# SeekStorm/SeekStorm

Measured on NVIDIA B200. Metric: queries/sec at top-10 (1M x 768 f32 cosine brute-force kNN), higher is better.
Workload: dtype f32

## Files before the change

### include/seekstorm_b200.h

```cpp
#ifndef SEEKSTORM_B200_H
#define SEEKSTORM_B200_H
#include <stdint.h>
#include <stddef.h>

#ifdef __cplusplus
extern "C" {
#endif

#define SSB_ABI_VERSION 3
#define SSB_K_MAX 32u
#define SSB_K_LIMIT 1024u
#define SSB_MAX_QUERY_TERMS 32u

enum { SSB_OK = 0, SSB_E_INVALID = -1, SSB_E_CUDA = -2, SSB_E_NOMEM = -3, SSB_E_STATE = -4,
       SSB_E_UNSUPPORTED = -5, SSB_E_NO_DEVICE = -6 };

enum { SSB_QUERY_UNION = 0, SSB_QUERY_INTERSECTION = 1, SSB_QUERY_PHRASE = 2 };
enum { SSB_RESULT_COUNT = 0, SSB_RESULT_TOPK = 1, SSB_RESULT_TOPKCOUNT = 2 };
enum { SSB_SIM_DOT = 0, SSB_SIM_COSINE = 1, SSB_SIM_EUCLIDEAN = 2 };
enum { SSB_QUANT_NONE = 0, SSB_QUANT_SCALAR_I8 = 1,
       SSB_QUANT_TURBO_I8 = 2 };
enum { SSB_VEC_KERNEL_AUTO = 0, SSB_VEC_KERNEL_FFMA = 1, SSB_VEC_KERNEL_TCGEN05 = 2, SSB_VEC_KERNEL_TCGEN05_N64 = 3,
       SSB_VEC_KERNEL_TCGEN05_BF16 = 4, SSB_VEC_KERNEL_TCGEN05_BF16_N64 = 5,
       SSB_VEC_KERNEL_TCGEN05_BF16_N256 = 6 ,
// ... 132 lines not shown
#define SSB_COMM_ID_BYTES 128
int32_t ssb_comm_unique_id(uint8_t* id128);
int32_t ssb_comm_init(ssb_index* ix, const uint8_t* id128, uint32_t rank, uint32_t world);
int32_t ssb_comm_attach(ssb_index* ix, void* nccl_comm, uint32_t rank, uint32_t world);
int32_t ssb_comm_destroy(ssb_index* ix);
int32_t ssb_lexical_sync_df(ssb_index* ix);

int32_t ssb_sync(ssb_index* ix);
void*   ssb_stream(ssb_index* ix);
#define SSB_OWN_STREAM ((void*)(intptr_t)-1)
int32_t ssb_set_stream(ssb_index* ix, void* cuda_stream);

typedef struct {
    uint64_t kernel_launches;
    uint64_t algorithmic_bytes;
    uint64_t h2d_bytes, d2h_bytes;
    uint64_t postings_visited;
    uint64_t probes;
    uint64_t items_processed;
    uint64_t items_skipped;
    uint64_t dominant_kernel_ns;
    uint64_t scan_bytes_read;
    uint64_t filter_fallbacks;
    uint64_t reserved[1];
} ssb_stats;
int32_t ssb_last_stats(const ssb_index* ix, ssb_stats* out);

#ifdef __cplusplus
}
#endif
#endif
```

### seekstorm_b200/_lib.py

```python
from __future__ import annotations

import ctypes as C
import os

_HERE = os.path.dirname(os.path.abspath(__file__))
LIB_PATH = os.environ.get("SSB_LIB") or os.path.join(_HERE, "libseekstorm_b200.so")

SSB_OK = 0
K_MAX = 32
MAX_QUERY_TERMS = 32

QUERY_UNION, QUERY_INTERSECTION, QUERY_PHRASE = 0, 1, 2
RESULT_COUNT, RESULT_TOPK, RESULT_TOPKCOUNT = 0, 1, 2
SIM_DOT, SIM_COSINE, SIM_EUCLIDEAN = 0, 1, 2


class SsbHit(C.Structure):
    _fields_ = [("doc_id", C.c_uint64), ("score", C.c_float), ("pad", C.c_uint32)]


class SsbConfig(C.Structure):
    _fields_ = [("device", C.c_int32), ("max_batch", C.c_uint32), ("vector_dims", C.c_uint32),
                ("vector_similarity", C.c_uint32), ("vector_kernel", C.c_uint32), ("vector_quantization", C.c_uint32),
                ("reserved", C.c_uint32 * 2)]


class SsbHitExt(C.Structure):
    _fields_ = [("field_id", C.c_uint32), ("chunk_id", C.c_uint32), ("level_id", C.c_uint32), ("shard_id", C.c_uint32),
                ("cluster_id", C.c_uint32), ("cluster_score", C.c_float), ("vector_score", C.c_float),
                ("lexical_score", C.c_float), ("source", C.c_uint32), ("pad", C.c_uint32 * 3)]


class SsbVecQuery(C.Structure):
# ... 18 lines not shown
                ("term_keys", C.c_void_p), ("term_flags", C.c_void_p),
                ("filter_offsets", C.c_void_p), ("filters", C.c_void_p), ("filter_set_values", C.c_void_p),
                ("field_masks", C.c_void_p)]


class SsbFacetField(C.Structure):
    _fields_ = [("type", C.c_uint32), ("offset", C.c_uint32)]


class SsbFacetFilter(C.Structure):
    _fields_ = [("facet", C.c_uint32), ("kind", C.c_uint32), ("start", C.c_uint64), ("end", C.c_uint64),
                ("set_first", C.c_uint32), ("set_count", C.c_uint32)]


FACET_U8, FACET_U16, FACET_U32, FACET_U64, FACET_I8, FACET_I16, FACET_I32, FACET_I64, FACET_TIMESTAMP, FACET_F32, FACET_F64, \
    FACET_STRING16, FACET_STRING32 = range(13)
FILTER_RANGE, FILTER_SET = 0, 1


class SsbStats(C.Structure):
    _fields_ = [("kernel_launches", C.c_uint64), ("algorithmic_bytes", C.c_uint64), ("h2d_bytes", C.c_uint64),
                ("d2h_bytes", C.c_uint64), ("postings_visited", C.c_uint64), ("probes", C.c_uint64),
                ("items_processed", C.c_uint64), ("items_skipped", C.c_uint64), ("dominant_kernel_ns", C.c_uint64),
                ("scan_bytes_read", C.c_uint64), ("filter_fallbacks", C.c_uint64), ("reserved", C.c_uint64 * 1)]


EXPORTS = [
    "ssb_abi_version", "ssb_last_error", "ssb_create", "ssb_destroy", "ssb_lexical_add_level",
    "ssb_vector_add_level_clustered", "ssb_lexical_set_field_boosts", "ssb_lexical_commit", "ssb_lexical_dict_size", "ssb_lexical_dict_export", "ssb_lexical_set_global_df",
    "ssb_load_index_bin", "ssb_load_vector_bin", "ssb_index_bin_inspect", "ssb_set_deleted", "ssb_set_facets", "ssb_vector_set_turboquant_mask", "ssb_vector_add_level", "ssb_vector_count", "ssb_vector_reserve", "ssb_set_vector_kernel", "ssb_search_lexical", "ssb_search_vector", "ssb_search_vector_ex", "ssb_search_hybrid",
    "ssb_rrf_fuse", "ssb_comm_unique_id", "ssb_comm_init", "ssb_comm_attach", "ssb_comm_destroy", "ssb_lexical_sync_df",
    "ssb_search_vector_keys", "ssb_search_lexical_keys", "ssb_merge_keys", "ssb_sync",
    "ssb_stream", "ssb_set_stream", "ssb_last_stats",
]

_lib = None


class SsbError(RuntimeError):
    pass


def lib():
    global _lib
    if _lib is not None:
        return _lib
    if not os.path.exists(LIB_PATH):
# ... 57 lines not shown
```

### seekstorm_b200/csrc/api.cu

```cuda
#include <stdarg.h>
#include <string.h>
#include <algorithm>
#include <condition_variable>
#include <exception>
#include <memory>
#include <mutex>
#include <new>
#include <shared_mutex>
#include <vector>

#include "bm25.h"
#include "comm.h"
#include "common.cuh"
#include "vec_scan.h"

namespace ssb {

static thread_local char g_err[512] = "";

void set_error(const char* fmt, ...) {
    va_list ap; va_start(ap, fmt);
    vsnprintf(g_err, sizeof(g_err), fmt, ap);
    va_end(ap);
}
// ... 200 lines not shown
        SSB_TRY(c.qlo.reserve((size_t)nq_pad * ix->dpad, 0, st));
        if (filter) SSB_TRY(c.q_scale.reserve(nq_pad, 0, st));
        SSB_TRY(vec::launch_prep_split_queries_bf16((const float*)qsrc, nq, ix->dims, ix->dims, c.qhi.p, c.qlo.p, nq_pad, ix->dpad,
                                                    ix->cfg.vector_similarity == SSB_SIM_COSINE, st, (filter || ivf) ? c.qpad.p : nullptr,
                                                    filter ? c.q_scale.p : nullptr, filter ? ix->vec_err.p : nullptr));
    } else
    SSB_TRY(vec::launch_prep_queries((const float*)qsrc, nq, ix->dims, ix->dims, c.qpad.p, nq_pad, ix->dpad,
                                     ix->cfg.vector_similarity == SSB_SIM_COSINE, st));
    c.stats.kernel_launches += 1;
    if (ix->n_rows == 0) { SSB_CUDA_TRY(cudaMemsetAsync(keys_out_dev, 0, (size_t)nq * LIST * 8, st)); return SSB_OK; }
    size_t sb = use_tc ? vec::scan_tc_scratch_bytes(ix->n_sms, nq_pad) : vec::scan_scratch_bytes(ix->n_sms, nq_pad);
    const size_t head_words = sb / 8 + (size_t)nq_pad * LIST + (nq_pad + 1) / 2;
    SSB_TRY(c.scratch.reserve(head_words + (filter ? vec::refine_scratch_words(ix->n_sms, nq_pad) : 0), 0, st));
    vec::ScanArgs a{};
    a.rows = ix->rows.p; a.rows_hi = ix->rows_hi.p; a.rows_lo = ix->rows_lo.p; a.rows_h16 = ix->rows_h16.p; a.doc_ids = ix->doc_ids.p; a.n_rows = ix->n_rows; a.dpad = ix->dpad; a.queries_padded = c.qpad.p;
    a.nq_pad = nq_pad; a.nq_valid = nq; a.k = k; a.similarity = ix->cfg.vector_similarity; a.n_sms = ix->n_sms;
    a.scratch = c.scratch.p; a.scratch_bytes = sb;
    uint64_t* merged = c.scratch.p + sb / 8;
    a.keys_out = merged; a.ev0 = c.ev0; a.ev1 = c.ev1; c.ev_used = true;
    a.thr_buf = reinterpret_cast<uint32_t*>(merged + (size_t)nq_pad * LIST);
    a.ceil_keys = ceil_dev;
    if (ix->del.n) { a.del_slot = ix->del.d_slot; a.del_words = ix->del.d_words; }
    a.launches = &c.stats.kernel_launches;
    if (ivf) {
        vec::IvfArgs v{};
        v.medoids = ix->medoids.p; v.lvl_begin = ix->lvl_begin.p; v.cl_count = ix->cl_count.p;
        v.n_clusters = ix->n_clusters; v.n_levels = (uint32_t)ix->h_lvl_begin.size(); v.max_level_clusters = ix->max_level_clusters;
        v.queries_padded = c.qpad.p; v.nq = nq; v.nq_pad = nq_pad; v.dpad = ix->dpad; v.similarity = ix->cfg.vector_similarity;
        v.ann_mode = ivf->mode; v.n_probe = ivf->n_probe; v.cluster_threshold = ivf->thr;
        v.words = (ix->n_clusters + 31) / 32;
        SSB_TRY(c.ivf_scores.reserve((size_t)nq * ix->n_clusters, 0, st));
        SSB_TRY(c.ivf_sel.reserve((size_t)nq_pad * v.words, 0, st));
        SSB_TRY(c.ivf_obs.reserve(nq, 0, st));
        v.scores = c.ivf_scores.p; v.sel = c.ivf_sel.p; v.observed = c.ivf_obs.p; v.launches = &c.stats.kernel_launches;
        SSB_TRY(vec::launch_ivf_select(v, st));
        a.ivf_sel = c.ivf_sel.p; a.ivf_words = v.words; a.row_cluster = ix->row_cluster.p;
    }
    if (ix->quant_i8) {
        a.rows_i8 = ix->rows_i8.p; a.queries_i8 = c.q_i8.p; a.dpad8 = ix->dpad8;
        if (ix->turbo || ix->cfg.vector_similarity != SSB_SIM_COSINE) {
            a.i8_scaled = ix->cfg.vector_similarity == SSB_SIM_EUCLIDEAN ? (ix->affine ? 3 : 2) : 1;
            a.row_aff = ix->row_aff.p; a.q_aff = c.q_aff.p;
            a.row_scale = ix->row_scale.p; a.row_norm = ix->row_norm.p; a.q_scale = c.q_scale.p; a.q_norm = c.q_norm.p;
        }
        SSB_TRY(vec::launch_scan_tc(a, 128, 2, st));
    } else if (use_tc) {
        SSB_TRY(c.qhi.reserve((size_t)nq_pad * ix->dpad, 0, st));
        SSB_TRY(c.qlo.reserve((size_t)nq_pad * ix->dpad, 0, st));
        a.q_hi = c.qhi.p; a.q_lo = c.qlo.p;
        if (filter) a.q_scale = c.q_scale.p;
        SSB_TRY(vec::launch_scan_tc(a, qt, filter ? (kern == SSB_VEC_KERNEL_TCGEN05_FILTER_N256_PAIR ? 4 : 3) : (tc_bf16 ? 1 : 0), st));
        if (filter) {
            vec::RefineArgs r{};
            r.rows = ix->rows.p; r.doc_ids = ix->doc_ids.p; r.n_rows = ix->n_rows; r.dpad = ix->dpad; r.queries_padded = c.qpad.p; r.margin = c.q_scale.p;
            r.keys = merged; r.keys_out = keys_out_dev;
            r.nq = nq; r.nq_pad = nq_pad; r.k = k;
            r.fb_lists = c.scratch.p + head_words;
            r.fb_state = reinterpret_cast<uint32_t*>(r.fb_lists + (size_t)nq_pad * ix->n_sms * LIST);
            r.del_slot = a.del_slot; r.del_words = a.del_words; r.ivf_sel = a.ivf_sel; r.ivf_words = a.ivf_words; r.row_cluster = a.row_cluster; r.n_sms = ix->n_sms; r.launches = &c.stats.kernel_launches;
            SSB_TRY(vec::launch_refine(r, st));
            c.fb_state = r.fb_state;
        }
    } else {
        SSB_TRY(vec::launch_scan_ffma(a, st));
    }
    if (!filter) SSB_CUDA_TRY(cudaMemcpyAsync(keys_out_dev, merged, (size_t)nq * LIST * 8, cudaMemcpyDeviceToDevice, st));
    c.stats.algorithmic_bytes += (uint64_t)(nq_pad / qt) * ix->n_rows * ix->dims * (ix->quant_i8 ? 1 : 4);
    c.stats.scan_bytes_read += filter ? (uint64_t)(nq_pad / qt) * ix->n_rows * ix->dims * 2 + (uint64_t)nq * LIST * ix->dims * 4
                                      : (uint64_t)(nq_pad / qt) * ix->n_rows * ix->dims * (ix->quant_i8 ? 1 : 4);
    return SSB_OK;
}

uint32_t decode_list(const uint64_t* keys, uint32_t k, ssb_hit* hits, bool dedup) {
    uint32_t n = 0;
    for (uint32_t j = 0; j < LIST && n < k; j++) {
        const uint64_t key = keys[j];
        if (!key) break;
        const uint64_t doc = key_doc(key);
        if (dedup) { bool seen = false; for (uint32_t i = 0; i < n; i++) seen = seen || hits[i].doc_id == doc; if (seen) continue; }
        hits[n].doc_id = doc; hits[n].score = key_score(key); hits[n].pad = 0;
        n++;
    }
    return n;
}

void decode_keys(const uint64_t* keys, uint32_t nq, uint32_t k, ssb_hit* hits, uint32_t* n_hits, bool dedup = false) {
    for (uint32_t q = 0; q < nq; q++) {
        const uint32_t n = decode_list(keys + (size_t)q * LIST, k, hits + (size_t)q * k, dedup);
        for (uint32_t j = n; j < k; j++) { hits[(size_t)q * k + j].doc_id = 0; hits[(size_t)q * k + j].score = 0.f; hits[(size_t)q * k + j].pad = 0; }
// ... 895 lines not shown
```

### seekstorm_b200/csrc/vec_refine.cu

```cuda
#include "common.cuh"
#include "vec_scan.h"

namespace ssb {
namespace vec {
namespace rf {

constexpr int RTHREADS = 128;
constexpr int QF = 4;
constexpr int FTHREADS = 256;

__device__ __forceinline__ float dot4(const float4 a, const float4 b, float s) {
    s = fmaf(a.x, b.x, s); s = fmaf(a.y, b.y, s); s = fmaf(a.z, b.z, s); return fmaf(a.w, b.w, s);
}

__global__ void __launch_bounds__(RTHREADS)
refine_candidates(const float* __restrict__ rows, const uint32_t* __restrict__ doc_ids, uint32_t dpad, const float* __restrict__ queries,
                  const float* __restrict__ margin, const uint64_t* keys, uint64_t* keys_out, uint32_t k, uint32_t* __restrict__ fb_state) {
    __shared__ uint64_t ex[LIST];
    const int warp = threadIdx.x >> 5, lane = threadIdx.x & 31;
    const uint32_t q = blockIdx.x;
    const uint64_t mine = keys[(size_t)q * LIST + lane];
    const float* qv = queries + (size_t)q * dpad;
    uint64_t ck[8]; const float* rp[8]; float s[8];
#pragma unroll
    for (int c = 0; c < 8; c++) {
        ck[c] = shfl64(mine, warp * 8 + c);
        rp[c] = rows + (size_t)(ck[c] ? key_doc(ck[c]) : 0u) * dpad;
        s[c] = 0.f;
    }
    if (ck[0]) {
        for (uint32_t i = lane * 4; i < dpad; i += 128) {
            const float4 b = *reinterpret_cast<const float4*>(qv + i);
#pragma unroll
            for (int c = 0; c < 8; c++) s[c] = dot4(__ldg(reinterpret_cast<const float4*>(rp[c] + i)), b, s[c]);
        }
    }
#pragma unroll
    for (int c = 0; c < 8; c++) {
        float v = s[c];
        for (int m = 16; m; m >>= 1) v += __shfl_xor_sync(FULL, v, m);
        if (lane == 0) {
            uint64_t key = 0;
            if (ck[c] && v == v) { const uint32_t row = key_doc(ck[c]); key = pack_key(v, doc_ids ? __ldg(&doc_ids[row]) : row); }
            ex[warp * 8 + c] = key;
        }
    }
    __syncthreads();
    if (warp == 0) {
        keys_out[(size_t)q * LIST + lane] = wl_sort_desc(ex[lane], lane);
        const uint64_t kth = shfl64(mine, (int)k - 1), last = shfl64(mine, LIST - 1);
        if (lane == 0 && last && kth) {
            const float m = margin[q], th = __fsub_rd(key_score(kth), m);
            if (!(m == m) || key_score(last) >= th) fb_state[1 + atomicAdd(&fb_state[0], 1u)] = q;
        }
    }
}

__global__ void __launch_bounds__(FTHREADS)
fallback_scan(const float* __restrict__ rows, const uint32_t* __restrict__ doc_ids, uint64_t n_rows, uint32_t dpad,
              const float* __restrict__ queries, const uint32_t* __restrict__ fb_state, uint64_t* __restrict__ fb_lists ,
              uint32_t k, const uint32_t* __restrict__ del_slot, const uint64_t* __restrict__ del_words,
              const uint32_t* __restrict__ ivf_sel, uint32_t ivf_words, const uint32_t* __restrict__ row_cluster) {
    const uint32_t nf = fb_state[0];
    if (nf == 0) return;
    extern __shared__ __align__(16) float qs[];
    __shared__ uint64_t sm[FTHREADS / 32][QF][LIST];
    const int warp = threadIdx.x >> 5, lane = threadIdx.x & 31;
    for (uint32_t base = 0; base < nf; base += QF) {
        for (uint32_t i = threadIdx.x; i < QF * dpad; i += FTHREADS) {
            const uint32_t j = i / dpad;
            qs[i] = base + j < nf ? queries[(size_t)fb_state[1 + base + j] * dpad + (i - j * dpad)] : 0.f;
        }
        __syncthreads();
        uint64_t L[QF];
#pragma unroll
        for (int j = 0; j < QF; j++) L[j] = 0;
        for (uint64_t row = (uint64_t)blockIdx.x * (FTHREADS / 32) + warp; row < n_rows; row += (uint64_t)gridDim.x * (FTHREADS / 32)) {
// ... 31 lines not shown
}

__global__ void __launch_bounds__(32)
fallback_merge(const uint32_t* __restrict__ fb_state, const uint64_t* __restrict__ fb_lists, uint32_t n_lists, uint64_t* __restrict__ keys) {
    const uint32_t nf = fb_state[0];
    const int lane = threadIdx.x;
    for (uint32_t slot = blockIdx.x; slot < nf; slot += gridDim.x) {
        uint64_t L = 0;
        for (uint32_t l = 0; l < n_lists; l++) {
            const uint64_t B = fb_lists[((size_t)slot * n_lists + l) * LIST + lane];
            if (__any_sync(FULL, B != 0)) L = wl_merge(L, B, lane);
        }
        keys[(size_t)fb_state[1 + slot] * LIST + lane] = L;
    }
}

}

size_t refine_scratch_words(int n_sms, uint32_t nq_pad) { return (size_t)nq_pad * (size_t)n_sms * LIST + (nq_pad + 2) / 2 + 1; }

int32_t launch_refine(const RefineArgs& a, cudaStream_t st) {
    if (a.nq == 0) return SSB_OK;
    SSB_CUDA_TRY(cudaMemsetAsync(a.fb_state, 0, 4, st));
    rf::refine_candidates<<<a.nq, rf::RTHREADS, 0, st>>>(a.rows, a.doc_ids, a.dpad, a.queries_padded, a.margin, a.keys, a.keys_out, a.k, a.fb_state);
    SSB_CUDA_TRY(cudaGetLastError());
    const int smem = rf::QF * (int)a.dpad * 4;
    if (smem > 200 * 1024) { set_error("filter scan: vector_dims too large for the fallback scan"); return SSB_E_UNSUPPORTED; }
    if (smem > 40 * 1024) SSB_CUDA_TRY(cudaFuncSetAttribute(rf::fallback_scan, cudaFuncAttributeMaxDynamicSharedMemorySize, smem));
    rf::fallback_scan<<<a.n_sms, rf::FTHREADS, smem, st>>>(a.rows, a.doc_ids, a.n_rows, a.dpad, a.queries_padded, a.fb_state, a.fb_lists, a.k,
                                                           a.del_slot, a.del_words, a.ivf_sel, a.ivf_words, a.row_cluster);
    SSB_CUDA_TRY(cudaGetLastError());
    rf::fallback_merge<<<64, 32, 0, st>>>(a.fb_state, a.fb_lists, (uint32_t)a.n_sms, a.keys_out);
    SSB_CUDA_TRY(cudaGetLastError());
    if (a.launches) *a.launches += 3;
    return SSB_OK;
}

}
}
```

### seekstorm_b200/csrc/vec_scan.h

```cpp
#pragma once
#include <cuda_runtime.h>
#include <stdint.h>

namespace ssb {
namespace vec {

constexpr int VEC_QT = 16;

struct ScanArgs {
    const float* rows;
    const void* rows_hi = nullptr; const void* rows_lo = nullptr;
    const void* rows_h16 = nullptr;
    const uint32_t* doc_ids;
    uint64_t n_rows;
    uint32_t dpad;
    const float* queries_padded;
    uint32_t nq_pad;
    uint32_t nq_valid = 0;
    uint32_t k;
    uint32_t similarity;
    int n_sms;
    uint64_t* scratch;
    size_t scratch_bytes;
    uint64_t* keys_out;
    cudaEvent_t ev0 = nullptr, ev1 = nullptr;
    float* q_hi = nullptr; float* q_lo = nullptr;
    uint32_t* thr_buf = nullptr;
    const uint32_t* thr_init = nullptr;
    const uint64_t* ceil_keys = nullptr;
    uint64_t* launches = nullptr;
    const int8_t* rows_i8 = nullptr;
    const int8_t* queries_i8 = nullptr;
    uint32_t dpad8 = 0;
    int i8_scaled = 0;
    const float* row_scale = nullptr; const float* row_norm = nullptr;
    const float* q_scale = nullptr; const float* q_norm = nullptr;
    const int* row_aff = nullptr; const int* q_aff = nullptr;
    const uint32_t* del_slot = nullptr; const uint64_t* del_words = nullptr;
    bool sample_groupmax = false;
    const uint32_t* ivf_sel = nullptr; uint32_t ivf_words = 0; const uint32_t* row_cluster = nullptr;
};

inline uint64_t vec_presample_rows(uint64_t n_rows, bool tensor_core) {
    if (n_rows < 65536) return 0;
    uint64_t s = tensor_core ? n_rows / 128 : n_rows / 32;
    const uint64_t lo = tensor_core ? 2048 : 4096, hi = tensor_core ? 8192 : 32768;
    s = s < lo ? lo : (s > hi ? hi : s);
    return s / 512 * 512;
}

int32_t launch_scan_ffma(const ScanArgs& a, cudaStream_t st);
size_t scan_scratch_bytes(int n_sms, uint32_t nq_pad);
int32_t launch_scan_tc(const ScanArgs& a, uint32_t nq_tile , int prec , cudaStream_t st);
size_t scan_tc_scratch_bytes(int n_sms, uint32_t nq_pad);
int32_t launch_prep_split_queries_bf16(const float* q, uint32_t nq, uint32_t dims, uint64_t qstride, void* hi, void* lo, uint32_t nq_pad,
                                       uint32_t dpad, int normalize, cudaStream_t st, float* f32_out = nullptr, float* margin_out = nullptr,
                                       const uint32_t* row_err = nullptr);
int32_t launch_rows_f16_err(const float* rows, void* h16, uint64_t n, uint32_t dpad, float scale, uint32_t* err, cudaStream_t st);
int32_t launch_max_abs_f32(const float* x, size_t n, uint32_t* out_bits, cudaStream_t st);
struct RefineArgs {
    const float* rows; const uint32_t* doc_ids; uint64_t n_rows; uint32_t dpad;
    const float* queries_padded;
    const float* margin;
    const uint64_t* keys;
    uint64_t* keys_out;
    uint32_t nq, nq_pad, k;
    uint32_t* fb_state;
    uint64_t* fb_lists;
    const uint32_t* del_slot; const uint64_t* del_words;
    const uint32_t* ivf_sel; uint32_t ivf_words; const uint32_t* row_cluster;
    int n_sms;
    uint64_t* launches;
};
struct IvfArgs {
    const float* medoids;
    const uint32_t* lvl_begin;
    const uint32_t* cl_count;
    uint32_t n_clusters, n_levels, max_level_clusters;
    const float* queries_padded;
    uint32_t nq, nq_pad, dpad, similarity;
    uint32_t ann_mode, n_probe; float cluster_threshold;
    float* scores;
    uint32_t* sel; uint32_t words;
    uint64_t* observed;
    uint64_t* launches;
};
int32_t launch_ivf_select(const IvfArgs& a, cudaStream_t st);
// ... 26 lines not shown
```

### seekstorm_b200/csrc/vec_scan_tc.cu

```cuda
#include <cuda_bf16.h>
#include <stdlib.h>
#include <cuda_fp16.h>

#include "common.cuh"
#include "vec_scan.h"

namespace ssb {
namespace vec {

namespace tc {
constexpr int KC = 32;
constexpr int TM = 128;
constexpr int MT = 2;
constexpr int TROWS = TM * MT;
constexpr int A1_BYTES = TM * KC * 4;
constexpr int A_BYTES = MT * A1_BYTES;
constexpr int THREADS = 512;
constexpr int SPLIT_THREADS = 256;
constexpr int CHUNK = 8;
enum { PREC_TF32 = 0, PREC_BF16 = 1, PREC_I8 = 2, PREC_F16F = 3 };

constexpr int MAX_STAGES = 6;
template <int NQ, int PREC, bool BRES = false> struct Cfg {
    static constexpr int MT = NQ == 256 ? 1 : 2;
// ... 576 lines not shown
                        else while (pm) { const int src = __ffs(pm) - 1; pm &= pm - 1; wl_insert(L, shfl64(key, src), lane); }
                        mylists[q * LIST + lane] = L;
                        uint32_t kth = (uint32_t)(shfl64(L, (int)k - 1) >> 32);
                        if (kth) kth = ord_f32(__fsub_rd(unord_f32(kth), qs_sm[q]));
                        if (lane == 0 && kth > thr_u[q]) atomicMax(&thr_u[q], kth);
                    }
                }
            }
            tc_fence_before();
            __syncwarp();
            if (lane == 0) mbar_arrive_leader(&tempty[buf]);
        }
    }

    tc_fence_before();
    __syncthreads();
    cluster_sync_all();
    if (warp == 1) {
        tc_fence_after();
        asm volatile("tcgen05.dealloc.cta_group::2.sync.aligned.b32 %0, %1;" ::"r"(tmem_base), "r"((uint32_t)C::TMEM_COLS) : "memory");
    }
}

__global__ void split_queries_tf32(const float* __restrict__ q, float* __restrict__ hi, float* __restrict__ lo, size_t n) {
    size_t i = (size_t)blockIdx.x * blockDim.x + threadIdx.x;
    if (i >= n) return;
    uint32_t x = __float_as_uint(q[i]), h = x & 0xFFFFE000u;
    hi[i] = __uint_as_float(h);
    lo[i] = __uint_as_float(x) - __uint_as_float(h);
}
__global__ void prep_split_queries_bf16(const float* __restrict__ q, uint32_t nq, uint32_t dims, uint64_t qstride,
                                        __nv_bfloat16* __restrict__ hi, __nv_bfloat16* __restrict__ lo, uint32_t nq_pad, uint32_t dpad, int normalize,
                                        float* __restrict__ f32_out ,
                                        float* __restrict__ margin_out , const uint32_t* __restrict__ row_err ) {
    const int lane = threadIdx.x & 31;
    const uint32_t row = blockIdx.x * (blockDim.x >> 5) + (threadIdx.x >> 5);
    if (row >= nq_pad) return;
    const bool filter = margin_out != nullptr;
    __nv_bfloat16* oh = hi + (size_t)row * dpad;
    __nv_bfloat16* ol = lo + (size_t)row * dpad;
    __half* o16 = reinterpret_cast<__half*>(oh);
    float* of = f32_out ? f32_out + (size_t)row * dpad : nullptr;
    if (row >= nq) {
        for (uint32_t i = lane; i < dpad; i += 32) { oh[i] = __float2bfloat16_rn(0.f); if (!filter) ol[i] = __float2bfloat16_rn(0.f); if (of) of[i] = 0.f; }
        if (filter && lane == 0) margin_out[row] = 0.f;
        return;
// ... 178 lines not shown
    SSB_TRY(encode_tmap_2d(&tmB, a.q_hi, 2, a.dpad, a.nq_pad, (uint64_t)a.dpad * 2, 64, C::NQH, 128));
    const uint32_t n_kchunks = (a.dpad + 63) / 64, n_groups = a.nq_pad / C::NQ;
    const uint32_t n_pairs = (uint32_t)((a.n_rows + 2 * tc::TM - 1) / (2 * tc::TM));
    uint32_t n_clusters = (uint32_t)a.n_sms / 2;
    if (n_clusters > n_pairs) n_clusters = n_pairs;
    const uint32_t gx = 2 * n_clusters;
    if ((size_t)n_groups * gx * 4 * C::NQ * LIST * 8 > a.scratch_bytes) { set_error("vector scan scratch too small"); return SSB_E_STATE; }
    SSB_CUDA_TRY(cudaFuncSetAttribute(tc::scan_tc2, cudaFuncAttributeMaxDynamicSharedMemorySize, C::SMEM));
    cudaLaunchConfig_t cfg{};
    cfg.gridDim = dim3(gx, n_groups); cfg.blockDim = dim3(tc::THREADS); cfg.dynamicSmemBytes = C::SMEM; cfg.stream = st;
    cudaLaunchAttribute at[1];
    at[0].id = cudaLaunchAttributeClusterDimension; at[0].val.clusterDim.x = 2; at[0].val.clusterDim.y = 1; at[0].val.clusterDim.z = 1;
    cfg.attrs = at; cfg.numAttrs = 1;
    if (a.ev0) cudaEventRecord(a.ev0, st);
    SSB_CUDA_TRY(cudaLaunchKernelEx(&cfg, tc::scan_tc2, tmA, tmB, (uint32_t)a.n_rows, n_kchunks, n_pairs, a.k, a.doc_ids, a.scratch, a.thr_init,
                                    a.nq_valid ? a.nq_valid : a.nq_pad, a.del_slot, a.del_words, a.q_scale, a.ivf_sel, a.ivf_words, a.row_cluster));
    if (a.ev1) cudaEventRecord(a.ev1, st);
    merge_lists_generic(a.scratch, gx * 4, C::NQ, a.nq_pad, a.keys_out, st);
    SSB_CUDA_TRY(cudaGetLastError());
    if (a.launches) *a.launches += 2;
    return SSB_OK;
}

static int32_t launch_scan_tc_impl(const ScanArgs& a, uint32_t nq_tile, int prec , cudaStream_t st) {
    if (a.n_rows == 0 || a.nq_pad == 0) return SSB_OK;
    if (prec == 4) return a.sample_groupmax ? launch_tc_n<256, tc::PREC_F16F>(a, st) : launch_tc2(a, st);
    if (prec == 2) {
        if (nq_tile != 128 || a.nq_pad % 128 != 0 || !a.rows_i8 || !a.queries_i8 || a.dpad8 % 128) { set_error("int8 scan: bad arguments"); return SSB_E_INVALID; }
        if (a.i8_scaled) {
            if (!a.row_scale || !a.q_scale || (a.i8_scaled >= 2 && (!a.row_norm || !a.q_norm)) || (a.i8_scaled == 3 && (!a.row_aff || !a.q_aff))) { set_error("scaled int8 scan: missing scale / norm arrays"); return SSB_E_INVALID; }
            if (a.i8_scaled == 3) return a.dpad8 <= 1024 ? launch_tc_n<128, tc::PREC_I8, true, 3>(a, st) : launch_tc_n<128, tc::PREC_I8, false, 3>(a, st);
            if (a.i8_scaled == 1) return a.dpad8 <= 1024 ? launch_tc_n<128, tc::PREC_I8, true, 1>(a, st) : launch_tc_n<128, tc::PREC_I8, false, 1>(a, st);
            return a.dpad8 <= 1024 ? launch_tc_n<128, tc::PREC_I8, true, 2>(a, st) : launch_tc_n<128, tc::PREC_I8, false, 2>(a, st);
        }
        return a.dpad8 <= 1024 ? launch_tc_n<128, tc::PREC_I8, true>(a, st) : launch_tc_n<128, tc::PREC_I8, false>(a, st);
    }
    if (a.similarity == SSB_SIM_EUCLIDEAN) { set_error("tcgen05 scan supports Dot/Cosine only"); return SSB_E_UNSUPPORTED; }
    if (prec == 3) {
        if ((nq_tile != 128 && nq_tile != 256) || a.nq_pad % nq_tile != 0) { set_error("tcgen05 filter scan: query count must be padded to the 128/256 query tile"); return SSB_E_INVALID; }
        return nq_tile == 256 ? launch_tc_n<256, tc::PREC_F16F>(a, st) : launch_tc_n<128, tc::PREC_F16F>(a, st);
    }
    if ((nq_tile != 64 && nq_tile != 128 && !(nq_tile == 256 && prec == 1)) || a.nq_pad % nq_tile != 0) { set_error("tcgen05 scan: query count must be padded to the 64/128(/256 bf16) query tile"); return SSB_E_INVALID; }
    if (prec == 1) return nq_tile == 64 ? launch_tc_n<64, tc::PREC_BF16>(a, st) : (nq_tile == 256 ? launch_tc_n<256, tc::PREC_BF16>(a, st) : launch_tc_n<128, tc::PREC_BF16>(a, st));
    return nq_tile == 64 ? launch_tc_n<64, tc::PREC_TF32>(a, st) : launch_tc_n<128, tc::PREC_TF32>(a, st);
}

int32_t launch_scan_tc(const ScanArgs& a, uint32_t nq_tile, int prec, cudaStream_t st) {
    if (a.thr_init || !a.thr_buf || a.del_slot || a.ivf_sel || vec_presample_rows(a.n_rows, true) == 0) return launch_scan_tc_impl(a, nq_tile, prec, st);
    ScanArgs pre = a;
    const uint64_t trows = nq_tile == 256 ? 128 : tc::TROWS;
    static const int env_tiles = [] { const char* e = getenv("SSB_TC_SAMPLE_TILES"); return e ? atoi(e) : 0; }();
    const int sample_tiles = env_tiles > 0 ? (env_tiles > 16 ? 16 : env_tiles) : ((prec >= 3 && nq_tile == 256) ? 2 : 1);
    uint64_t s = (uint64_t)a.n_sms * trows * sample_tiles;
    if (s > a.n_rows / 4) s = a.n_rows / 4 / trows * trows;
    pre.n_rows = s; pre.ev0 = nullptr; pre.ev1 = nullptr;
    pre.sample_groupmax = true;
    SSB_TRY(launch_scan_tc_impl(pre, nq_tile, prec, st));
    ScanArgs full = a;
    full.thr_init = a.thr_buf;
    return launch_scan_tc_impl(full, nq_tile, prec, st);
}

void launch_kth_from_groupmax(const void* gmax, uint32_t n_groups, uint32_t nq, uint32_t k, uint32_t* thr, int is_int, cudaStream_t st) {
    if (nq) tc::kth_from_groupmax<<<nq, 256, 0, st>>>((const int*)gmax, n_groups, nq, k, thr, is_int, nullptr);
}

int32_t launch_prep_split_queries_bf16(const float* q, uint32_t nq, uint32_t dims, uint64_t qstride, void* hi, void* lo, uint32_t nq_pad,
                                       uint32_t dpad, int normalize, cudaStream_t st, float* f32_out, float* margin_out, const uint32_t* row_err) {
    if (nq_pad == 0) return SSB_OK;
    tc::prep_split_queries_bf16<<<(nq_pad + 7) / 8, 256, 0, st>>>(q, nq, dims, qstride, (__nv_bfloat16*)hi, (__nv_bfloat16*)lo, nq_pad, dpad, normalize,
                                                                  f32_out, margin_out, row_err);
    SSB_CUDA_TRY(cudaGetLastError());
    return SSB_OK;
}

int32_t launch_split_rows_bf16(const float* rows, void* hi, void* lo, size_t n_elems, cudaStream_t st) {
    if (n_elems == 0) return SSB_OK;
    tc::split_rows_bf16<<<(unsigned)((n_elems + 255) / 256), 256, 0, st>>>(rows, (__nv_bfloat16*)hi, (__nv_bfloat16*)lo, n_elems);
// ... 22 lines not shown
```

### seekstorm_b200/index.py

```python
from __future__ import annotations

import ctypes as C
import enum
from dataclasses import dataclass, field
from typing import Callable, Optional, Sequence

import numpy as np

from . import _lib
from ._lib import SsbConfig, SsbHit, SsbLevelDesc, SsbLexBatch, SsbStats, check, lib


class QueryType(enum.IntEnum):
    Union = 0
    Intersection = 1
    Phrase = 2


class ResultType(enum.IntEnum):
    Count = 0
    Topk = 1
    TopkCount = 2


# ... 371 lines not shown
        return out, ext, observed[:nq]

    def search_hybrid_batch(self, queries_keys, query_type: QueryType, queries, k: int):
        nq = len(queries_keys)
        b, keep = self._lex_batch(queries_keys, query_type)
        if isinstance(queries, np.ndarray):
            queries = np.ascontiguousarray(queries, dtype=np.float32)
        hits = _hits_array(max(nq * k, 1))
        n_hits = np.zeros(max(nq, 1), dtype=np.uint32)
        check(lib().ssb_search_hybrid(self._h, C.byref(b), _addr(queries), k, hits.ctypes.data, n_hits.ctypes.data))
        out = []
        for i in range(nq):
            h = hits[i * k: i * k + int(n_hits[i])]
            out.append([(int(d), float(s)) for d, s in zip(h["doc_id"], h["score"])])
        return out

    def last_stats(self) -> dict:
        s = SsbStats()
        check(lib().ssb_last_stats(self._h, C.byref(s)))
        return dict(kernel_launches=s.kernel_launches, algorithmic_bytes=s.algorithmic_bytes, h2d_bytes=s.h2d_bytes,
                    d2h_bytes=s.d2h_bytes, postings_visited=s.postings_visited, probes=s.probes,
                    items_processed=s.items_processed, items_skipped=s.items_skipped,
                    dominant_kernel_ns=s.dominant_kernel_ns, scan_bytes_read=s.scan_bytes_read,
                    filter_fallbacks=s.filter_fallbacks)

    def search_vector_keys(self, queries_dev, k: int, keys_out_dev):
        check(lib().ssb_search_vector_keys(self._h, _addr(queries_dev), int(queries_dev.shape[0]), k, _addr(keys_out_dev)))

    def search_lexical_keys(self, batch_struct, k: int, result_type: ResultType, keys_out_dev, counts_dev=None):
        check(lib().ssb_search_lexical_keys(self._h, C.byref(batch_struct), k, int(result_type), _addr(keys_out_dev),
                                            _addr(counts_dev)))

    def merge_keys(self, keys_dev, n_lists: int, nq: int, k: int):
        hits = _hits_array(max(nq * k, 1))
        n_hits = np.zeros(max(nq, 1), dtype=np.uint32)
        check(lib().ssb_merge_keys(self._h, _addr(keys_dev), n_lists, nq, k, hits.ctypes.data, n_hits.ctypes.data))
        return [[(int(d), float(s)) for d, s in zip(hits[i * k: i * k + int(n_hits[i])]["doc_id"],
                                                     hits[i * k: i * k + int(n_hits[i])]["score"])] for i in range(nq)]

    def merge_keys_raw(self, keys_dev, n_lists: int, nq: int, k: int, hits, n_hits):
        check(lib().ssb_merge_keys(self._h, _addr(keys_dev), n_lists, nq, k, hits.ctypes.data, n_hits.ctypes.data))

    def sync(self):
        check(lib().ssb_sync(self._h))

    @property
    def stream(self) -> int:
# ... 84 lines not shown
```

Before: 534,300.

## Add paired-CTA tcgen05 filter scan with queries resident in TMEM and threshold candidate lists

Adds a new fp16 filter-scan kernel for the pair path. A 2-CTA cluster keeps the query tile in tensor memory as the A operand and streams only the fp16 row plane through a deep TMA pipeline. The epilogue no longer keeps a per-query top list; it appends every score above a presampled threshold to a per-query candidate buffer using atomics, and the refine kernel rebuilds the top list from those candidates. The aim is to cut shared-memory traffic for queries and the cost of top-k maintenance. In exchange, atomics can contend, and a candidate cap that overflows sends the query to the fallback path.

```diff
diff --git a/include/seekstorm_b200.h b/include/seekstorm_b200.h
--- a/include/seekstorm_b200.h
+++ b/include/seekstorm_b200.h
@@ -178,8 +178,9 @@
     uint64_t dominant_kernel_ns;
     uint64_t scan_bytes_read;
     uint64_t filter_fallbacks;
-    uint64_t reserved[1];
+    uint64_t scan_kernel;
 } ssb_stats;
+enum { SSB_SCAN_FFMA = 1, SSB_SCAN_TC = 2, SSB_SCAN_TC2 = 3, SSB_SCAN_TC2Q = 4 };
 int32_t ssb_last_stats(const ssb_index* ix, ssb_stats* out);
 
 #ifdef __cplusplus
diff --git a/seekstorm_b200/_lib.py b/seekstorm_b200/_lib.py
--- a/seekstorm_b200/_lib.py
+++ b/seekstorm_b200/_lib.py
@@ -9,6 +9,7 @@
 SSB_OK = 0
 K_MAX = 32
 MAX_QUERY_TERMS = 32
+SCAN_FFMA, SCAN_TC, SCAN_TC2, SCAN_TC2Q = 1, 2, 3, 4
 
 QUERY_UNION, QUERY_INTERSECTION, QUERY_PHRASE = 0, 1, 2
 RESULT_COUNT, RESULT_TOPK, RESULT_TOPKCOUNT = 0, 1, 2
@@ -73,7 +74,7 @@
     _fields_ = [("kernel_launches", C.c_uint64), ("algorithmic_bytes", C.c_uint64), ("h2d_bytes", C.c_uint64),
                 ("d2h_bytes", C.c_uint64), ("postings_visited", C.c_uint64), ("probes", C.c_uint64),
                 ("items_processed", C.c_uint64), ("items_skipped", C.c_uint64), ("dominant_kernel_ns", C.c_uint64),
-                ("scan_bytes_read", C.c_uint64), ("filter_fallbacks", C.c_uint64), ("reserved", C.c_uint64 * 1)]
+                ("scan_bytes_read", C.c_uint64), ("filter_fallbacks", C.c_uint64), ("scan_kernel", C.c_uint64)]
 
 
 EXPORTS = [
diff --git a/seekstorm_b200/csrc/api.cu b/seekstorm_b200/csrc/api.cu
--- a/seekstorm_b200/csrc/api.cu
+++ b/seekstorm_b200/csrc/api.cu
@@ -246,6 +246,8 @@
     a.ceil_keys = ceil_dev;
     if (ix->del.n) { a.del_slot = ix->del.d_slot; a.del_words = ix->del.d_words; }
     a.launches = &c.stats.kernel_launches;
+    vec::ScanInfo info{};
+    a.info = &info;
     if (ivf) {
         vec::IvfArgs v{};
         v.medoids = ix->medoids.p; v.lvl_begin = ix->lvl_begin.p; v.cl_count = ix->cl_count.p;
@@ -278,6 +280,7 @@
             vec::RefineArgs r{};
             r.rows = ix->rows.p; r.doc_ids = ix->doc_ids.p; r.n_rows = ix->n_rows; r.dpad = ix->dpad; r.queries_padded = c.qpad.p; r.margin = c.q_scale.p;
             r.keys = merged; r.keys_out = keys_out_dev;
+            r.cand = info.cand; r.cand_cnt = info.cand_cnt; r.cand_cap = info.cand_cap;
             r.nq = nq; r.nq_pad = nq_pad; r.k = k;
             r.fb_lists = c.scratch.p + head_words;
             r.fb_state = reinterpret_cast<uint32_t*>(r.fb_lists + (size_t)nq_pad * ix->n_sms * LIST);
@@ -289,6 +292,7 @@
         SSB_TRY(vec::launch_scan_ffma(a, st));
     }
     if (!filter) SSB_CUDA_TRY(cudaMemcpyAsync(keys_out_dev, merged, (size_t)nq * LIST * 8, cudaMemcpyDeviceToDevice, st));
+    c.stats.scan_kernel = info.kernel ? info.kernel : (use_tc ? SSB_SCAN_TC : SSB_SCAN_FFMA);
     c.stats.algorithmic_bytes += (uint64_t)(nq_pad / qt) * ix->n_rows * ix->dims * (ix->quant_i8 ? 1 : 4);
     c.stats.scan_bytes_read += filter ? (uint64_t)(nq_pad / qt) * ix->n_rows * ix->dims * 2 + (uint64_t)nq * LIST * ix->dims * 4
                                       : (uint64_t)(nq_pad / qt) * ix->n_rows * ix->dims * (ix->quant_i8 ? 1 : 4);
diff --git a/seekstorm_b200/csrc/vec_refine.cu b/seekstorm_b200/csrc/vec_refine.cu
--- a/seekstorm_b200/csrc/vec_refine.cu
+++ b/seekstorm_b200/csrc/vec_refine.cu
@@ -15,11 +15,30 @@
 
 __global__ void __launch_bounds__(RTHREADS)
 refine_candidates(const float* __restrict__ rows, const uint32_t* __restrict__ doc_ids, uint32_t dpad, const float* __restrict__ queries,
-                  const float* __restrict__ margin, const uint64_t* keys, uint64_t* keys_out, uint32_t k, uint32_t* __restrict__ fb_state) {
+                  const float* __restrict__ margin, const uint64_t* keys, uint64_t* keys_out, uint32_t k, uint32_t* __restrict__ fb_state,
+                  const uint64_t* __restrict__ cand, const uint32_t* __restrict__ cand_cnt, uint32_t cap) {
     __shared__ uint64_t ex[LIST];
+    __shared__ uint64_t sel[RTHREADS / 32][LIST];
     const int warp = threadIdx.x >> 5, lane = threadIdx.x & 31;
     const uint32_t q = blockIdx.x;
-    const uint64_t mine = keys[(size_t)q * LIST + lane];
+    uint64_t mine;
+    bool over = false;
+    if (cand) {
+        const uint32_t n = cand_cnt[q], m = n < cap ? n : cap;
+        over = n > cap;
+        const uint64_t* cq = cand + (size_t)q * cap;
+        uint64_t L = 0;
+        for (uint32_t b = warp * 32; b < m; b += RTHREADS) {
+            const uint64_t key = b + lane < m ? cq[b + lane] : 0ull;
+            if (__any_sync(FULL, key > shfl64(L, LIST - 1))) L = wl_merge(L, wl_sort_desc(key, lane), lane);
+        }
+        sel[warp][lane] = L;
+        __syncthreads();
+        mine = sel[0][lane];
+        for (int w = 1; w < RTHREADS / 32; w++) mine = wl_merge(mine, sel[w][lane], lane);
+    } else {
+        mine = keys[(size_t)q * LIST + lane];
+    }
     const float* qv = queries + (size_t)q * dpad;
     uint64_t ck[8]; const float* rp[8]; float s[8];
 #pragma unroll
@@ -49,10 +68,12 @@
     if (warp == 0) {
         keys_out[(size_t)q * LIST + lane] = wl_sort_desc(ex[lane], lane);
         const uint64_t kth = shfl64(mine, (int)k - 1), last = shfl64(mine, LIST - 1);
-        if (lane == 0 && last && kth) {
+        bool flag = over;
+        if (last && kth) {
             const float m = margin[q], th = __fsub_rd(key_score(kth), m);
-            if (!(m == m) || key_score(last) >= th) fb_state[1 + atomicAdd(&fb_state[0], 1u)] = q;
+            flag = flag || !(m == m) || key_score(last) >= th;
         }
+        if (lane == 0 && flag) fb_state[1 + atomicAdd(&fb_state[0], 1u)] = q;
     }
 }
 
@@ -130,7 +151,8 @@
 int32_t launch_refine(const RefineArgs& a, cudaStream_t st) {
     if (a.nq == 0) return SSB_OK;
     SSB_CUDA_TRY(cudaMemsetAsync(a.fb_state, 0, 4, st));
-    rf::refine_candidates<<<a.nq, rf::RTHREADS, 0, st>>>(a.rows, a.doc_ids, a.dpad, a.queries_padded, a.margin, a.keys, a.keys_out, a.k, a.fb_state);
+    rf::refine_candidates<<<a.nq, rf::RTHREADS, 0, st>>>(a.rows, a.doc_ids, a.dpad, a.queries_padded, a.margin, a.keys, a.keys_out, a.k, a.fb_state,
+                                                   a.cand, a.cand_cnt, a.cand_cap);
     SSB_CUDA_TRY(cudaGetLastError());
     const int smem = rf::QF * (int)a.dpad * 4;
     if (smem > 200 * 1024) { set_error("filter scan: vector_dims too large for the fallback scan"); return SSB_E_UNSUPPORTED; }
diff --git a/seekstorm_b200/csrc/vec_scan.h b/seekstorm_b200/csrc/vec_scan.h
--- a/seekstorm_b200/csrc/vec_scan.h
+++ b/seekstorm_b200/csrc/vec_scan.h
@@ -6,6 +6,11 @@
 namespace vec {
 
 constexpr int VEC_QT = 16;
+
+struct ScanInfo {
+    uint32_t kernel = 0;
+    const uint64_t* cand = nullptr; const uint32_t* cand_cnt = nullptr; uint32_t cand_cap = 0;
+};
 
 struct ScanArgs {
     const float* rows;
@@ -39,6 +44,7 @@
     const uint32_t* del_slot = nullptr; const uint64_t* del_words = nullptr;
     bool sample_groupmax = false;
     const uint32_t* ivf_sel = nullptr; uint32_t ivf_words = 0; const uint32_t* row_cluster = nullptr;
+    ScanInfo* info = nullptr;
 };
 
 inline uint64_t vec_presample_rows(uint64_t n_rows, bool tensor_core) {
@@ -63,6 +69,7 @@
     const float* queries_padded;
     const float* margin;
     const uint64_t* keys;
+    const uint64_t* cand = nullptr; const uint32_t* cand_cnt = nullptr; uint32_t cand_cap = 0;
     uint64_t* keys_out;
     uint32_t nq, nq_pad, k;
     uint32_t* fb_state;
diff --git a/seekstorm_b200/csrc/vec_scan_tc.cu b/seekstorm_b200/csrc/vec_scan_tc.cu
--- a/seekstorm_b200/csrc/vec_scan_tc.cu
+++ b/seekstorm_b200/csrc/vec_scan_tc.cu
@@ -622,6 +622,155 @@
     }
 }
 
+struct Cfg2q {
+    static constexpr int NQ = 256, NQH = 128;
+    static constexpr int NT = 64, NTH = 32;
+    static constexpr int STAGE_BYTES = NTH * 128;
+    static constexpr int STAGES = 48;
+    static constexpr int SMEM = STAGES * STAGE_BYTES + (2 * STAGES + 4) * 8 + 16;
+    static constexpr int TMEM_COLS = 512;
+    static constexpr int D_COLS = 2 * NT;
+    static constexpr int MAX_KCHUNKS = (TMEM_COLS - D_COLS) / 32;
+    static constexpr int THREADS = 384;
+    static constexpr int EPI_WARPS = 8;
+};
+
+__global__ void __launch_bounds__(Cfg2q::THREADS, 1)
+scan_tc2q(const __grid_constant__ CUtensorMap tmA, const __half* __restrict__ q_h16 , uint32_t dpad, uint32_t n_rows,
+          uint32_t n_kchunks, uint32_t n_ptiles, const uint32_t* __restrict__ thr_init, uint32_t nq_valid,
+          uint64_t* __restrict__ cand , uint32_t* __restrict__ cnt , uint32_t cap) {
+    using C = Cfg2q;
+    extern __shared__ __align__(1024) uint8_t base[];
+    uint8_t* stage0 = base;
+    uint64_t* full = (uint64_t*)(base + C::STAGES * C::STAGE_BYTES);
+    uint64_t* empty = full + C::STAGES;
+    uint64_t* tfull = empty + C::STAGES;
+    uint64_t* tempty = tfull + 2;
+    uint32_t* tmem_slot = (uint32_t*)(tempty + 2);
+
+    const int warp = threadIdx.x >> 5, lane = threadIdx.x & 31;
+    const uint32_t rank = cluster_ctarank();
+    const uint32_t pair0 = blockIdx.x >> 1, n_clusters = gridDim.x >> 1;
+
+    if (threadIdx.x == 0) {
+        for (int s = 0; s < C::STAGES; s++) { mbar_init(&full[s], 1); mbar_init(&empty[s], 1); }
+        for (int b = 0; b < 2; b++) { mbar_init(&tfull[b], 1); mbar_init(&tempty[b], 2 * C::EPI_WARPS); }
+        fence_mbar_init();
+    }
+    if (warp == 1) {
+        asm volatile("tcgen05.alloc.cta_group::2.sync.aligned.shared::cta.b32 [%0], %1;" ::"r"(smem_u32(tmem_slot)), "r"((uint32_t)C::TMEM_COLS) : "memory");
+        asm volatile("tcgen05.relinquish_alloc_permit.cta_group::2.sync.aligned;" ::: "memory");
+    }
+    tc_fence_before();
+    __syncthreads();
+    tc_fence_after();
+    const uint32_t tmem_base = *(volatile uint32_t*)tmem_slot;
+    const int ew = warp & 3, eg = (warp - 4) >> 2;
+    const uint32_t q = blockIdx.y * C::NQ + rank * C::NQH + (uint32_t)(ew * 32 + lane);
+    if (warp >= 4) {
+        const uint4* src = reinterpret_cast<const uint4*>(q_h16 + (size_t)q * dpad);
+        const uint32_t taddr = tmem_base + ((uint32_t)(ew * 32) << 16) + C::D_COLS;
+        for (uint32_t b = eg; b < n_kchunks * 2; b += 2) {
+            uint4 v[4] = {};
+            if (b * 32 < dpad) {
+#pragma unroll
+                for (int i = 0; i < 4; i++) v[i] = __ldg(src + b * 4 + i);
+            }
+            asm volatile("tcgen05.st.sync.aligned.32x32b.x16.b32 [%0], {%1,%2,%3,%4,%5,%6,%7,%8,%9,%10,%11,%12,%13,%14,%15,%16};"
+                         ::"r"(taddr + b * 16), "r"(v[0].x), "r"(v[0].y), "r"(v[0].z), "r"(v[0].w), "r"(v[1].x), "r"(v[1].y), "r"(v[1].z), "r"(v[1].w),
+                           "r"(v[2].x), "r"(v[2].y), "r"(v[2].z), "r"(v[2].w), "r"(v[3].x), "r"(v[3].y), "r"(v[3].z), "r"(v[3].w) : "memory");
+        }
+        asm volatile("tcgen05.wait::st.sync.aligned;" ::: "memory");
+    }
+    tc_fence_before();
+    __syncthreads();
+    cluster_sync_all();
+    tc_fence_after();
+
+    if (warp == 0) {
+        if (lane == 0) {
+            tma_prefetch_desc(&tmA);
+            uint32_t it = 0;
+            for (uint32_t pt = pair0; pt < n_ptiles; pt += n_clusters) {
+                for (uint32_t kc = 0; kc < n_kchunks; ++kc, ++it) {
+                    const uint32_t s = it % C::STAGES, ph = (it / C::STAGES) & 1u;
+                    mbar_wait(&empty[s], ph ^ 1u);
+                    if (rank == 0) mbar_arrive_expect_tx(&full[s], 2 * C::STAGE_BYTES);
+                    tma_load_2d_pair(stage0 + s * C::STAGE_BYTES, &tmA, (int)(kc * 64), (int)(pt * C::NT + rank * C::NTH), &full[s]);
+                }
+            }
+        }
+    } else if (warp == 1) {
+        if (lane == 0 && rank == 0) {
+            const uint32_t idesc = (1u << 4) | (0u << 7) | (0u << 10) | ((uint32_t)(C::NT >> 3) << 17) | ((uint32_t)(C::NQ >> 4) << 24);
+            uint32_t it = 0, ti = 0;
+            for (uint32_t pt = pair0; pt < n_ptiles; pt += n_clusters, ++ti) {
+                const uint32_t buf = ti & 1u, tph = (ti >> 1) & 1u;
+                mbar_wait(&tempty[buf], tph ^ 1u);
+                tc_fence_after();
+                const uint32_t d = tmem_base + buf * C::NT;
+                for (uint32_t kc = 0; kc < n_kchunks; ++kc, ++it) {
+                    const uint32_t s = it % C::STAGES, ph = (it / C::STAGES) & 1u;
+                    mbar_wait(&full[s], ph);
+                    tc_fence_after();
+                    const uint64_t b = umma_desc_k128(smem_u32(stage0 + s * C::STAGE_BYTES));
+                    const uint32_t a = tmem_base + C::D_COLS + kc * 32;
+#pragma unroll
+                    for (uint32_t kk = 0; kk < 4; kk++)
+                        asm volatile("{\n.reg .pred p;\nsetp.ne.b32 p, %4, 0;\ntcgen05.mma.cta_group::2.kind::f16 [%0], [%1], %2, %3, p;\n}\n"
+                                     ::"r"(d), "r"(a + kk * 8), "l"(b + (uint64_t)(kk * 2)), "r"(idesc), "r"((uint32_t)((kc | kk) != 0)) : "memory");
+                    umma_commit_pair(&empty[s]);
+                    if (kc + 1 == n_kchunks) umma_commit_pair(&tfull[buf]);
+                }
+            }
+        }
+    } else if (warp >= 4) {
+        const uint32_t thr = q < nq_valid ? __ldg(&thr_init[q]) : 0xFFFFFFFFu;
+        uint64_t* my = cand + (size_t)q * cap;
+        uint32_t ti = 0;
+        for (uint32_t pt = pair0; pt < n_ptiles; pt += n_clusters, ++ti) {
+            const uint32_t buf = ti & 1u, tph = (ti >> 1) & 1u;
+            mbar_wait(&tfull[buf], tph);
+            tc_fence_after();
+            uint32_t v[32];
+            const uint32_t taddr = tmem_base + ((uint32_t)(ew * 32) << 16) + buf * C::NT + eg * 32;
+            asm volatile("tcgen05.ld.sync.aligned.32x32b.x32.b32 {%0,%1,%2,%3,%4,%5,%6,%7,%8,%9,%10,%11,%12,%13,%14,%15,"
+                         "%16,%17,%18,%19,%20,%21,%22,%23,%24,%25,%26,%27,%28,%29,%30,%31}, [%32];"
+                         : "=r"(v[0]), "=r"(v[1]), "=r"(v[2]), "=r"(v[3]), "=r"(v[4]), "=r"(v[5]), "=r"(v[6]), "=r"(v[7]),
+                           "=r"(v[8]), "=r"(v[9]), "=r"(v[10]), "=r"(v[11]), "=r"(v[12]), "=r"(v[13]), "=r"(v[14]), "=r"(v[15]),
+                           "=r"(v[16]), "=r"(v[17]), "=r"(v[18]), "=r"(v[19]), "=r"(v[20]), "=r"(v[21]), "=r"(v[22]), "=r"(v[23]),
+                           "=r"(v[24]), "=r"(v[25]), "=r"(v[26]), "=r"(v[27]), "=r"(v[28]), "=r"(v[29]), "=r"(v[30]), "=r"(v[31])
+                         : "r"(taddr) : "memory");
+            asm volatile("tcgen05.wait::ld.sync.aligned;" ::: "memory");
+            tc_fence_before();
+            __syncwarp();
+            if (lane == 0) mbar_arrive_leader(&tempty[buf]);
+            bool any = false;
+#pragma unroll
+            for (int j = 0; j < 32; j++) any |= ord_f32(__uint_as_float(v[j])) >= thr;
+            if (!any) continue;
+            const uint32_t row0 = pt * C::NT + (uint32_t)(eg * 32);
+#pragma unroll
+            for (int j = 0; j < 32; j++) {
+                const float sc = __uint_as_float(v[j]);
+                const uint32_t so = ord_f32(sc), row = row0 + (uint32_t)j;
+                if (row < n_rows && sc == sc && so >= thr) {
+                    const uint32_t slot = atomicAdd(&cnt[q], 1u);
+                    if (slot < cap) my[slot] = ((uint64_t)so << 32) | (uint64_t)(0xFFFFFFFFu - row);
+                }
+            }
+        }
+    }
+
+    tc_fence_before();
+    __syncthreads();
+    cluster_sync_all();
+    if (warp == 1) {
+        tc_fence_after();
+        asm volatile("tcgen05.dealloc.cta_group::2.sync.aligned.b32 %0, %1;" ::"r"(tmem_base), "r"((uint32_t)C::TMEM_COLS) : "memory");
+    }
+}
+
 __global__ void split_queries_tf32(const float* __restrict__ q, float* __restrict__ hi, float* __restrict__ lo, size_t n) {
     size_t i = (size_t)blockIdx.x * blockDim.x + threadIdx.x;
     if (i >= n) return;
@@ -846,9 +995,56 @@
     return SSB_OK;
 }
 
+static uint64_t tc_sample_rows(uint64_t n_rows, int n_sms, uint32_t nq_tile, int prec) {
+    const uint64_t trows = nq_tile == 256 ? 128 : tc::TROWS;
+    static const int env_tiles = [] { const char* e = getenv("SSB_TC_SAMPLE_TILES"); return e ? atoi(e) : 0; }();
+    const int sample_tiles = env_tiles > 0 ? (env_tiles > 16 ? 16 : env_tiles) : ((prec >= 3 && nq_tile == 256) ? 2 : 1);
+    uint64_t s = (uint64_t)n_sms * trows * sample_tiles;
+    if (s > n_rows / 4) s = n_rows / 4 / trows * trows;
+    return s;
+}
+
+static int32_t launch_tc2q(const ScanArgs& a, cudaStream_t st) {
+    using C = tc::Cfg2q;
+    if (a.nq_pad % C::NQ != 0) { set_error("tcgen05 pair scan: query count must be padded to 256"); return SSB_E_INVALID; }
+    CUtensorMap tmA;
+    SSB_TRY(encode_tmap_2d(&tmA, a.rows_h16, 2, a.dpad, a.n_rows, (uint64_t)a.dpad * 2, 64, C::NTH, 128));
+    const uint32_t n_kchunks = (a.dpad + 63) / 64, n_groups = a.nq_pad / C::NQ;
+    const uint32_t n_ptiles = (uint32_t)((a.n_rows + C::NT - 1) / C::NT);
+    uint32_t n_clusters = (uint32_t)a.n_sms / 2;
+    if (n_clusters > n_ptiles) n_clusters = n_ptiles;
+    const uint64_t s = tc_sample_rows(a.n_rows, a.n_sms, C::NQ, 4);
+    uint64_t cap = s ? (uint64_t)a.k * a.n_rows / s * 8 : 0;
+    if (cap < 1024) cap = 1024;
+    const uint64_t cap_max = (a.scratch_bytes - (size_t)a.nq_pad * 4) / ((size_t)a.nq_pad * 8);
+    if (cap > cap_max) cap = cap_max;
+    if (cap < 64) { set_error("vector scan scratch too small"); return SSB_E_STATE; }
+    uint32_t* cnt = reinterpret_cast<uint32_t*>(a.scratch + (size_t)a.nq_pad * cap);
+    SSB_CUDA_TRY(cudaMemsetAsync(cnt, 0, (size_t)a.nq_pad * 4, st));
+    SSB_CUDA_TRY(cudaFuncSetAttribute(tc::scan_tc2q, cudaFuncAttributeMaxDynamicSharedMemorySize, C::SMEM));
+    cudaLaunchConfig_t cfg{};
+    cfg.gridDim = dim3(2 * n_clusters, n_groups); cfg.blockDim = dim3(C::THREADS); cfg.dynamicSmemBytes = C::SMEM; cfg.stream = st;
+    cudaLaunchAttribute at[1];
+    at[0].id = cudaLaunchAttributeClusterDimension; at[0].val.clusterDim.x = 2; at[0].val.clusterDim.y = 1; at[0].val.clusterDim.z = 1;
+    cfg.attrs = at; cfg.numAttrs = 1;
+    if (a.ev0) cudaEventRecord(a.ev0, st);
+    SSB_CUDA_TRY(cudaLaunchKernelEx(&cfg, tc::scan_tc2q, tmA, (const __half*)a.q_hi, a.dpad, (uint32_t)a.n_rows, n_kchunks, n_ptiles, a.thr_init,
+                                    a.nq_valid ? a.nq_valid : a.nq_pad, a.scratch, cnt, (uint32_t)cap));
+    if (a.ev1) cudaEventRecord(a.ev1, st);
+    if (a.info) { a.info->kernel = SSB_SCAN_TC2Q; a.info->cand = a.scratch; a.info->cand_cnt = cnt; a.info->cand_cap = (uint32_t)cap; }
+    if (a.launches) *a.launches += 1;
+    return SSB_OK;
+}
+
 static int32_t launch_scan_tc_impl(const ScanArgs& a, uint32_t nq_tile, int prec , cudaStream_t st) {
     if (a.n_rows == 0 || a.nq_pad == 0) return SSB_OK;
-    if (prec == 4) return a.sample_groupmax ? launch_tc_n<256, tc::PREC_F16F>(a, st) : launch_tc2(a, st);
+    if (prec == 4) {
+        if (a.sample_groupmax) return launch_tc_n<256, tc::PREC_F16F>(a, st);
+        if (!a.rows_h16 || !a.q_scale) { set_error("tcgen05 filter scan: the index holds no fp16 plane / no margins"); return SSB_E_STATE; }
+        if (a.thr_init && a.info && (a.dpad + 63) / 64 <= (uint32_t)tc::Cfg2q::MAX_KCHUNKS) return launch_tc2q(a, st);
+        if (a.info) a.info->kernel = SSB_SCAN_TC2;
+        return launch_tc2(a, st);
+    }
     if (prec == 2) {
         if (nq_tile != 128 || a.nq_pad % 128 != 0 || !a.rows_i8 || !a.queries_i8 || a.dpad8 % 128) { set_error("int8 scan: bad arguments"); return SSB_E_INVALID; }
         if (a.i8_scaled) {
@@ -872,12 +1068,7 @@
 int32_t launch_scan_tc(const ScanArgs& a, uint32_t nq_tile, int prec, cudaStream_t st) {
     if (a.thr_init || !a.thr_buf || a.del_slot || a.ivf_sel || vec_presample_rows(a.n_rows, true) == 0) return launch_scan_tc_impl(a, nq_tile, prec, st);
     ScanArgs pre = a;
-    const uint64_t trows = nq_tile == 256 ? 128 : tc::TROWS;
-    static const int env_tiles = [] { const char* e = getenv("SSB_TC_SAMPLE_TILES"); return e ? atoi(e) : 0; }();
-    const int sample_tiles = env_tiles > 0 ? (env_tiles > 16 ? 16 : env_tiles) : ((prec >= 3 && nq_tile == 256) ? 2 : 1);
-    uint64_t s = (uint64_t)a.n_sms * trows * sample_tiles;
-    if (s > a.n_rows / 4) s = a.n_rows / 4 / trows * trows;
-    pre.n_rows = s; pre.ev0 = nullptr; pre.ev1 = nullptr;
+    pre.n_rows = tc_sample_rows(a.n_rows, a.n_sms, nq_tile, prec); pre.ev0 = nullptr; pre.ev1 = nullptr;
     pre.sample_groupmax = true;
     SSB_TRY(launch_scan_tc_impl(pre, nq_tile, prec, st));
     ScanArgs full = a;
diff --git a/seekstorm_b200/index.py b/seekstorm_b200/index.py
--- a/seekstorm_b200/index.py
+++ b/seekstorm_b200/index.py
@@ -417,7 +417,7 @@
                     d2h_bytes=s.d2h_bytes, postings_visited=s.postings_visited, probes=s.probes,
                     items_processed=s.items_processed, items_skipped=s.items_skipped,
                     dominant_kernel_ns=s.dominant_kernel_ns, scan_bytes_read=s.scan_bytes_read,
-                    filter_fallbacks=s.filter_fallbacks)
+                    filter_fallbacks=s.filter_fallbacks, scan_kernel=s.scan_kernel)
 
     def search_vector_keys(self, queries_dev, k: int, keys_out_dev):
         check(lib().ssb_search_vector_keys(self._h, _addr(queries_dev), int(queries_dev.shape[0]), k, _addr(keys_out_dev)))
```

Result: slower. 460,400, median of 6 (-13.8%).
